# christhetree/mod_extraction

Measured on AMD Instinct MI355X. Metric: 44.1 kHz audio-seconds/sec (train step), interwoven ph/fl/ch, higher is better.
Workload: dtype f32

## Files before the change

mod_extraction_amd/csrc/melspec.hip:

```cpp
#include "wave_fft.h"

#define MEL_NFFT 1024
#define MEL_FR 16

struct cfloat { float re, im; };
__device__ __forceinline__ cfloat cmul(cfloat a, cfloat b)
{
    cfloat r;
    r.re = a.re * b.re - a.im * b.im;
    r.im = a.re * b.im + a.im * b.re;
    return r;
}
__device__ __forceinline__ cfloat cadd(cfloat a, cfloat b) { return {a.re + b.re, a.im + b.im}; }
__device__ __forceinline__ cfloat csub(cfloat a, cfloat b) { return {a.re - b.re, a.im - b.im}; }

__global__ __launch_bounds__(256) void melspec_kernel(
    const float *__restrict__ x, int N, const float *__restrict__ window,
    const float2 *__restrict__ twiddle,
    const float *__restrict__ fb,
    const int *__restrict__ band_lo, const int *__restrict__ band_hi, int n_mels, int hop,
    int n_frames, int out_pitch, float eps, int f0, int f1, int t0, int t1, int coef_cap, float *__restrict__ out)
{
    __shared__ cfloat fftbuf[4][MEL_NFFT + 64];
    __shared__ float powbuf[4][MEL_NFFT / 2 + 1];
    __shared__ float2 tw_s[MEL_NFFT];
    extern __shared__ float melbuf[];
    const int tid = threadIdx.x, lane = tid & 63, wave = tid >> 6;
    const int plane = blockIdx.y;
    const int tile0 = blockIdx.x * MEL_FR;
    const float *xp = x + (size_t)plane * N;
    cfloat *buf = fftbuf[wave];
    float *power = powbuf[wave];
    float *coef = melbuf + n_mels * (MEL_FR + 1);
    int *boff = reinterpret_cast<int *>(coef + coef_cap);
    for (int i = tid; i < MEL_NFFT; i += 256) tw_s[i] = twiddle[i];
    if (tid == 0) {
        int acc = 0;
        for (int m = 0; m < n_mels; ++m) { boff[m] = acc; acc += band_hi[m] - band_lo[m]; }
        boff[n_mels] = acc;
    }
    __syncthreads();
    const bool packed = boff[n_mels] <= coef_cap;
    if (packed) {
        for (int m = tid; m < n_mels; m += 256) {
            const int lo = band_lo[m], hi = band_hi[m], o = boff[m];
            for (int kk = lo; kk < hi; ++kk) coef[o + kk - lo] = fb[(size_t)kk * n_mels + m];
        }
    }
    __syncthreads();

    for (int fl = wave; fl < MEL_FR; fl += 4) {
        const int t = tile0 + fl;
        if (t >= n_frames) continue;
        cfloat R[4][4];
#pragma unroll
        for (int bq = 0; bq < 4; ++bq)
#pragma unroll
            for (int cq = 0; cq < 4; ++cq) {
                const int n = lane + 64 * bq + 256 * cq;
                int sidx = t * hop + n - MEL_NFFT / 2;
                if (sidx < 0) sidx = -sidx;
                if (sidx >= N) sidx = 2 * (N - 1) - sidx;
                sidx = sidx < 0 ? 0 : sidx;
                R[bq][cq].re = xp[sidx] * window[n];
                R[bq][cq].im = 0.0f;
            }
        auto bfly = [&](int pass, int j, const cfloat (&vin)[4], cfloat (&o)[4]) {
            const int Ns = 1 << (2 * pass);
            const int k = j & (Ns - 1);
            const int tw_step = k * (MEL_NFFT / (Ns * 4));
            cfloat v0 = vin[0], v1 = vin[1], v2 = vin[2], v3 = vin[3];
            if (pass > 0) {
                float2 w1 = tw_s[tw_step], w2 = tw_s[2 * tw_step], w3 = tw_s[3 * tw_step];
                v1 = cmul(v1, {w1.x, w1.y});
                v2 = cmul(v2, {w2.x, w2.y});
                v3 = cmul(v3, {w3.x, w3.y});
            }
            cfloat a0 = cadd(v0, v2), a1 = csub(v0, v2), a2 = cadd(v1, v3), d = csub(v1, v3);
            cfloat a3 = {d.im, -d.re};
            o[0] = cadd(a0, a2);
            o[1] = cadd(a1, a3);
            o[2] = csub(a0, a2);
            o[3] = csub(a1, a3);
        };
        auto out_pos = [](int pass, int j, int r) {
            const int Ns = 1 << (2 * pass), k = j & (Ns - 1);
            return ((j - k) << 2) + k + r * Ns;
        };
        cfloat O[4][4], P[4][4];
#pragma unroll
        for (int bq = 0; bq < 4; ++bq) bfly(0, lane + 64 * bq, R[bq], O[bq]);
#pragma unroll
        for (int r = 0; r < 4; ++r) {
            const cfloat vin[4] = {O[0][r], O[1][r], O[2][r], O[3][r]};
            bfly(1, 4 * lane + r, vin, P[r]);
        }
#pragma unroll
        for (int r = 0; r < 4; ++r)
#pragma unroll
            for (int r2 = 0; r2 < 4; ++r2) {
                const int q = out_pos(1, 4 * lane + r, r2);
                buf[q + (q >> 4)] = P[r][r2];
            }
        __builtin_amdgcn_wave_barrier();
#pragma unroll
        for (int bq = 0; bq < 4; ++bq)
#pragma unroll
            for (int cq = 0; cq < 4; ++cq) {
                const int q = lane + 64 * bq + 256 * cq;
                R[bq][cq] = buf[q + (q >> 4)];
            }
        __builtin_amdgcn_wave_barrier();
        const int k2 = lane & 15;
#pragma unroll
        for (int bq = 0; bq < 4; ++bq) bfly(2, lane + 64 * bq, R[bq], O[bq]);
#pragma unroll
        for (int r = 0; r < 4; ++r) {
            const cfloat vin[4] = {O[0][r], O[1][r], O[2][r], O[3][r]};
            bfly(3, 4 * (lane - k2) + k2 + 16 * r, vin, P[r]);
        }
#pragma unroll
        for (int r = 0; r < 4; ++r)
#pragma unroll
            for (int r2 = 0; r2 < 4; ++r2) {
                const int q = out_pos(3, 4 * (lane - k2) + k2 + 16 * r, r2);
                buf[q + 16 * (q >> 8)] = P[r][r2];
            }
        __builtin_amdgcn_wave_barrier();
#pragma unroll
        for (int bq = 0; bq < 4; ++bq)
#pragma unroll
            for (int cq = 0; cq < 4; ++cq) {
                const int q = lane + 64 * bq + 256 * cq;
                R[bq][cq] = buf[q + 16 * (q >> 8)];
            }
        __builtin_amdgcn_wave_barrier();
#pragma unroll
        for (int bq = 0; bq < 4; ++bq) {
            const int j = lane + 64 * bq;
            bfly(4, j, R[bq], O[bq]);
#pragma unroll
            for (int r = 0; r < 3; ++r) {
                const int bin = j + 256 * r;
                if (bin <= MEL_NFFT / 2) {
                    const cfloat z = O[bq][r];
                    const float mag = sqrtf(z.re * z.re + z.im * z.im);
                    power[bin] = mag * mag;
                }
            }
        }
        __builtin_amdgcn_wave_barrier();
        for (int m = lane; m < n_mels; m += 64) {
            float acc = 0.0f;
            const int lo = band_lo[m], hi = band_hi[m];
            if (packed) {
                const float *cm = coef + boff[m] - lo;
                for (int kk = lo; kk < hi; ++kk) acc = fmaf(cm[kk], power[kk], acc);
            } else {
                float c = 0.0f;
                for (int kk = lo; kk < hi; ++kk) {
                    const float yv = fb[(size_t)kk * n_mels + m] * power[kk] - c;
                    const float tv = acc + yv;
                    c = (tv - acc) - yv;
                    acc = tv;
                }
            }
            melbuf[m * (MEL_FR + 1) + fl] = acc;
        }
        __builtin_amdgcn_wave_barrier();
    }
    __syncthreads();
    float *op = out + (size_t)plane * n_mels * out_pitch;
    for (int idx = tid; idx < n_mels * MEL_FR; idx += 256) {
        const int m = idx / MEL_FR, fl = idx % MEL_FR;
        const int t = tile0 + fl;
        if (t < out_pitch) {
            float v = 0.0f;
            if (t < n_frames) {
                float p = melbuf[m * (MEL_FR + 1) + fl];
                if ((m >= f0 && m < f1) || (t >= t0 && t < t1)) p = 0.0f;
                v = logf(fmaxf(p, eps));
            }
            op[(size_t)m * out_pitch + t] = v;
        }
    }
}

template <int NF>
__global__ __launch_bounds__(WF<NF>::WAVES * 64) void melspec_wf_kernel(
    const float *__restrict__ x, int N, const float *__restrict__ window, const float2 *__restrict__ twiddle,
    const float *__restrict__ fb, const int *__restrict__ band_lo, const int *__restrict__ band_hi, int n_mels, int hop,
    int n_frames, int out_pitch, float eps, int f0, int f1, int t0, int t1, int coef_cap, float *__restrict__ out)
{
    constexpr int L = WF<NF>::L, E = WF<NF>::E, NB = WF<NF>::NB, WAVES = WF<NF>::WAVES, FW = WF<NF>::FW, NT = WAVES * 64;
    __shared__ cf fftbuf[WAVES * FW][WF<NF>::LEN];
    __shared__ float powbuf[WAVES * FW][NF / 2 + 1];
    __shared__ cf tw_s[NF];
    extern __shared__ float melbuf[];
    const int tid = threadIdx.x, lane = tid & 63, wave = tid >> 6, g = lane / L, a = lane % L;
    const int plane = blockIdx.y;
    const int tile0 = blockIdx.x * MEL_FR;
    const float *xp = x + (size_t)plane * N;
    cf *buf = fftbuf[wave * FW + g];
    float *power = powbuf[wave * FW + g];
    float *coef = melbuf + n_mels * (MEL_FR + 1);
    int *boff = reinterpret_cast<int *>(coef + coef_cap);
    for (int i = tid; i < NF; i += NT) {
        const float2 w = twiddle[i];
        tw_s[i] = {w.x, w.y};
    }
    if (tid == 0) {
        int acc = 0;
        for (int m = 0; m < n_mels; ++m) { boff[m] = acc; acc += band_hi[m] - band_lo[m]; }
        boff[n_mels] = acc;
    }
    __syncthreads();
    const bool packed = boff[n_mels] <= coef_cap;
    if (packed) {
        for (int m = tid; m < n_mels; m += NT) {
            const int lo = band_lo[m], hi = band_hi[m], o = boff[m];
            for (int kk = lo; kk < hi; ++kk) coef[o + kk - lo] = fb[(size_t)kk * n_mels + m];
        }
    }
    __syncthreads();
    FftLane<NF> fl_;
    fft_lane_setup<NF, 1>(fl_, buf, tw_s, twiddle, a);

    for (int fb0 = wave * FW; fb0 < MEL_FR; fb0 += WAVES * FW) {
        const int fl = fb0 + g;
        if (tile0 + fb0 >= n_frames) break;
        const int t = tile0 + fl;
        const bool live = t < n_frames && fl < MEL_FR;
        const int tt = live ? t : n_frames - 1;
        cf R[NB][4], Z[E];
#pragma unroll
        for (int bq = 0; bq < NB; ++bq)
#pragma unroll
            for (int cq = 0; cq < 4; ++cq) {
                const int n = a + L * bq + (NF / 4) * cq;
                int sidx = tt * hop + n - NF / 2;
                if (sidx < 0) sidx = -sidx;
                if (sidx >= N) sidx = 2 * (N - 1) - sidx;
                sidx = sidx < 0 ? 0 : sidx;
                R[bq][cq] = {xp[sidx] * window[n], 0.0f};
            }
        wave_fft<NF, false>(R, Z, fl_);
#pragma unroll
        for (int i = 0; i < E; ++i) {
            const int bin = pos_final<NF>(i, a);
            if (bin <= NF / 2) {
                const float mag = sqrtf(Z[i].x * Z[i].x + Z[i].y * Z[i].y);
                power[bin] = mag * mag;
            }
        }
        __builtin_amdgcn_wave_barrier();
        if (live) {
            for (int m = a; m < n_mels; m += L) {
                float acc = 0.0f;
                const int lo = band_lo[m], hi = band_hi[m];
                if (packed) {
                    const float *cm = coef + boff[m] - lo;
                    for (int kk = lo; kk < hi; ++kk) acc = fmaf(cm[kk], power[kk], acc);
                } else {
                    float c = 0.0f;
                    for (int kk = lo; kk < hi; ++kk) {
                        const float yv = fb[(size_t)kk * n_mels + m] * power[kk] - c;
                        const float tv = acc + yv;
                        c = (tv - acc) - yv;
                        acc = tv;
                    }
                }
                melbuf[m * (MEL_FR + 1) + fl] = acc;
            }
        }
        __builtin_amdgcn_wave_barrier();
    }
    __syncthreads();
    float *op = out + (size_t)plane * n_mels * out_pitch;
    for (int idx = tid; idx < n_mels * MEL_FR; idx += NT) {
        const int m = idx / MEL_FR, fl = idx % MEL_FR;
        const int t = tile0 + fl;
        if (t < out_pitch) {
            float v = 0.0f;
            if (t < n_frames) {
                float p = melbuf[m * (MEL_FR + 1) + fl];
                if ((m >= f0 && m < f1) || (t >= t0 && t < t1)) p = 0.0f;
                v = logf(fmaxf(p, eps));
            }
            op[(size_t)m * out_pitch + t] = v;
        }
    }
}

MX_EXPORT int mx_logmel_fwd(const float *x, int64_t planes, int64_t N, const float *window,
                            const float *twiddle, const float *fb, const int32_t *band_lo,
                            const int32_t *band_hi, int64_t n_fft, int64_t hop, int64_t n_mels,
                            int64_t n_frames, int64_t out_pitch, float eps, int32_t f0, int32_t f1,
                            int32_t t0, int32_t t1, float *out, void *stream)
{
    if (!x || !window || !twiddle || !fb || !band_lo || !band_hi || !out || planes <= 0) return MX_ERR_ARG;
    if (hop <= 0 || n_frames < 0 || (N > 0 && n_frames > N / hop + 1)) return MX_ERR_ARG;
    if ((n_fft != 512 && n_fft != 1024 && n_fft != 2048) || N <= n_fft / 2 || N >= (1ll << 30) || planes > 65535 || n_mels > 2048 ||
        out_pitch < n_frames)
        return MX_ERR_UNSUPPORTED;
    const int tiles = (int)((out_pitch + MEL_FR - 1) / MEL_FR);
    const int coef_cap = 2 * ((int)n_fft / 2 + 1) + 2 * (int)n_mels;
    const size_t lds = ((size_t)n_mels * (MEL_FR + 1) + coef_cap + n_mels + 1) * sizeof(float);
    const void *fn = n_fft == MEL_NFFT ? (const void *)melspec_kernel
                     : n_fft == 512    ? (const void *)melspec_wf_kernel<512>
                                       : (const void *)melspec_wf_kernel<2048>;
    static size_t static_lds[3] = {0, 0, 0};
    static MxLdsLatch latch[3] = {};
    const int ki = n_fft == MEL_NFFT ? 0 : n_fft == 512 ? 1 : 2;
    if (!static_lds[ki]) {
        hipFuncAttributes fa;
        if (hipFuncGetAttributes(&fa, fn) != hipSuccess) return MX_ERR_LAUNCH;
        static_lds[ki] = fa.sharedSizeBytes ? fa.sharedSizeBytes : 1;
    }
    const size_t lds_cap = 160 * 1024;
    if (static_lds[ki] + lds > lds_cap) return MX_ERR_UNSUPPORTED;
    if (static_lds[ki] + lds > 64 * 1024 && mx_set_dyn_lds(latch[ki], fn, lds_cap - static_lds[ki]) != MX_OK) return MX_ERR_LAUNCH;
    if (n_fft != MEL_NFFT) {
        if (n_fft == 512)
            hipLaunchKernelGGL((melspec_wf_kernel<512>), dim3(tiles, (unsigned)planes), dim3(WF<512>::WAVES * 64), lds, (hipStream_t)stream,
                               x, (int)N, window, (const float2 *)twiddle, fb, band_lo, band_hi, (int)n_mels, (int)hop, (int)n_frames,
                               (int)out_pitch, eps, f0, f1, t0, t1, coef_cap, out);
        else
            hipLaunchKernelGGL((melspec_wf_kernel<2048>), dim3(tiles, (unsigned)planes), dim3(WF<2048>::WAVES * 64), lds, (hipStream_t)stream,
                               x, (int)N, window, (const float2 *)twiddle, fb, band_lo, band_hi, (int)n_mels, (int)hop, (int)n_frames,
                               (int)out_pitch, eps, f0, f1, t0, t1, coef_cap, out);
        return mx_launch_status();
    }
    hipLaunchKernelGGL(melspec_kernel, dim3(tiles, (unsigned)planes), dim3(256), lds, (hipStream_t)stream,
                       x, (int)N, window, (const float2 *)twiddle, fb, band_lo, band_hi, (int)n_mels, (int)hop,
                       (int)n_frames, (int)out_pitch, eps, f0, f1, t0, t1, coef_cap, out);
    return mx_launch_status();
}
```

Baseline: 7580.

## Process multiple mel tiles per workgroup and skip masked frames and bands

The 1024-point mel kernel now loops over several frame tiles per workgroup, chosen when the grid is large, so the per-block setup (twiddle load, band offsets, filterbank packing) is amortised. The serial prefix sum over band widths becomes a wave-level shuffle scan, and band limits are cached in LDS. Interior frames skip reflection index math, and the mel dot product is unrolled by four. Frames and mel bands inside the masked ranges skip FFT and dot work entirely. The trade-off is fewer workgroups, which lowers parallelism on smaller inputs, plus extra LDS and an unrolled loop that reads a few entries past each band.

```diff
diff --git a/mod_extraction_amd/csrc/melspec.hip b/mod_extraction_amd/csrc/melspec.hip
--- a/mod_extraction_amd/csrc/melspec.hip
+++ b/mod_extraction_amd/csrc/melspec.hip
@@ -2,6 +2,9 @@
 
 #define MEL_NFFT 1024
 #define MEL_FR 16
+#ifndef MEL_TPW
+#define MEL_TPW 2
+#endif
 
 struct cfloat { float re, im; };
 __device__ __forceinline__ cfloat cmul(cfloat a, cfloat b)
@@ -19,170 +22,223 @@
     const float2 *__restrict__ twiddle,
     const float *__restrict__ fb,
     const int *__restrict__ band_lo, const int *__restrict__ band_hi, int n_mels, int hop,
-    int n_frames, int out_pitch, float eps, int f0, int f1, int t0, int t1, int coef_cap, float *__restrict__ out)
+    int n_frames, int out_pitch, float eps, int f0, int f1, int t0, int t1, int coef_cap, int tiles_per_wg,
+    float *__restrict__ out)
 {
     __shared__ cfloat fftbuf[4][MEL_NFFT + 64];
-    __shared__ float powbuf[4][MEL_NFFT / 2 + 1];
+    __shared__ float powbuf[4][MEL_NFFT / 2 + 4];
     __shared__ float2 tw_s[MEL_NFFT];
     extern __shared__ float melbuf[];
     const int tid = threadIdx.x, lane = tid & 63, wave = tid >> 6;
     const int plane = blockIdx.y;
-    const int tile0 = blockIdx.x * MEL_FR;
     const float *xp = x + (size_t)plane * N;
     cfloat *buf = fftbuf[wave];
     float *power = powbuf[wave];
     float *coef = melbuf + n_mels * (MEL_FR + 1);
     int *boff = reinterpret_cast<int *>(coef + coef_cap);
+    int *blo = boff + n_mels + 1, *bhi = blo + n_mels;
     for (int i = tid; i < MEL_NFFT; i += 256) tw_s[i] = twiddle[i];
-    if (tid == 0) {
-        int acc = 0;
-        for (int m = 0; m < n_mels; ++m) { boff[m] = acc; acc += band_hi[m] - band_lo[m]; }
-        boff[n_mels] = acc;
+    for (int m = tid; m < n_mels; m += 256) {
+        blo[m] = band_lo[m];
+        bhi[m] = band_hi[m];
+    }
+    __syncthreads();
+    if (tid < 64) {
+        const int per = (n_mels + 63) / 64, m0 = lane * per, m1 = min(m0 + per, n_mels);
+        int s = 0;
+        for (int m = m0; m < m1; ++m) s += bhi[m] - blo[m];
+        int incl = s;
+#pragma unroll
+        for (int d = 1; d < 64; d <<= 1) {
+            const int v = __shfl_up(incl, d);
+            if (lane >= d) incl += v;
+        }
+        int acc = incl - s;
+        for (int m = m0; m < m1; ++m) { boff[m] = acc; acc += bhi[m] - blo[m]; }
+        if (lane == 63) boff[n_mels] = incl;
     }
     __syncthreads();
     const bool packed = boff[n_mels] <= coef_cap;
     if (packed) {
         for (int m = tid; m < n_mels; m += 256) {
-            const int lo = band_lo[m], hi = band_hi[m], o = boff[m];
-            for (int kk = lo; kk < hi; ++kk) coef[o + kk - lo] = fb[(size_t)kk * n_mels + m];
-        }
-    }
-    __syncthreads();
-
-    for (int fl = wave; fl < MEL_FR; fl += 4) {
-        const int t = tile0 + fl;
-        if (t >= n_frames) continue;
-        cfloat R[4][4];
-#pragma unroll
-        for (int bq = 0; bq < 4; ++bq)
-#pragma unroll
-            for (int cq = 0; cq < 4; ++cq) {
-                const int n = lane + 64 * bq + 256 * cq;
-                int sidx = t * hop + n - MEL_NFFT / 2;
-                if (sidx < 0) sidx = -sidx;
-                if (sidx >= N) sidx = 2 * (N - 1) - sidx;
-                sidx = sidx < 0 ? 0 : sidx;
-                R[bq][cq].re = xp[sidx] * window[n];
-                R[bq][cq].im = 0.0f;
-            }
-        auto bfly = [&](int pass, int j, const cfloat (&vin)[4], cfloat (&o)[4]) {
-            const int Ns = 1 << (2 * pass);
-            const int k = j & (Ns - 1);
-            const int tw_step = k * (MEL_NFFT / (Ns * 4));
-            cfloat v0 = vin[0], v1 = vin[1], v2 = vin[2], v3 = vin[3];
-            if (pass > 0) {
-                float2 w1 = tw_s[tw_step], w2 = tw_s[2 * tw_step], w3 = tw_s[3 * tw_step];
-                v1 = cmul(v1, {w1.x, w1.y});
-                v2 = cmul(v2, {w2.x, w2.y});
-                v3 = cmul(v3, {w3.x, w3.y});
-            }
-            cfloat a0 = cadd(v0, v2), a1 = csub(v0, v2), a2 = cadd(v1, v3), d = csub(v1, v3);
-            cfloat a3 = {d.im, -d.re};
-            o[0] = cadd(a0, a2);
-            o[1] = cadd(a1, a3);
-            o[2] = csub(a0, a2);
-            o[3] = csub(a1, a3);
-        };
-        auto out_pos = [](int pass, int j, int r) {
-            const int Ns = 1 << (2 * pass), k = j & (Ns - 1);
-            return ((j - k) << 2) + k + r * Ns;
-        };
-        cfloat O[4][4], P[4][4];
-#pragma unroll
-        for (int bq = 0; bq < 4; ++bq) bfly(0, lane + 64 * bq, R[bq], O[bq]);
-#pragma unroll
-        for (int r = 0; r < 4; ++r) {
-            const cfloat vin[4] = {O[0][r], O[1][r], O[2][r], O[3][r]};
-            bfly(1, 4 * lane + r, vin, P[r]);
-        }
-#pragma unroll
-        for (int r = 0; r < 4; ++r)
-#pragma unroll
-            for (int r2 = 0; r2 < 4; ++r2) {
-                const int q = out_pos(1, 4 * lane + r, r2);
-                buf[q + (q >> 4)] = P[r][r2];
-            }
-        __builtin_amdgcn_wave_barrier();
-#pragma unroll
-        for (int bq = 0; bq < 4; ++bq)
-#pragma unroll
-            for (int cq = 0; cq < 4; ++cq) {
-                const int q = lane + 64 * bq + 256 * cq;
-                R[bq][cq] = buf[q + (q >> 4)];
-            }
-        __builtin_amdgcn_wave_barrier();
-        const int k2 = lane & 15;
-#pragma unroll
-        for (int bq = 0; bq < 4; ++bq) bfly(2, lane + 64 * bq, R[bq], O[bq]);
-#pragma unroll
-        for (int r = 0; r < 4; ++r) {
-            const cfloat vin[4] = {O[0][r], O[1][r], O[2][r], O[3][r]};
-            bfly(3, 4 * (lane - k2) + k2 + 16 * r, vin, P[r]);
-        }
-#pragma unroll
-        for (int r = 0; r < 4; ++r)
-#pragma unroll
-            for (int r2 = 0; r2 < 4; ++r2) {
-                const int q = out_pos(3, 4 * (lane - k2) + k2 + 16 * r, r2);
-                buf[q + 16 * (q >> 8)] = P[r][r2];
-            }
-        __builtin_amdgcn_wave_barrier();
-#pragma unroll
-        for (int bq = 0; bq < 4; ++bq)
-#pragma unroll
-            for (int cq = 0; cq < 4; ++cq) {
-                const int q = lane + 64 * bq + 256 * cq;
-                R[bq][cq] = buf[q + 16 * (q >> 8)];
-            }
-        __builtin_amdgcn_wave_barrier();
-#pragma unroll
-        for (int bq = 0; bq < 4; ++bq) {
-            const int j = lane + 64 * bq;
-            bfly(4, j, R[bq], O[bq]);
-#pragma unroll
-            for (int r = 0; r < 3; ++r) {
-                const int bin = j + 256 * r;
-                if (bin <= MEL_NFFT / 2) {
-                    const cfloat z = O[bq][r];
-                    const float mag = sqrtf(z.re * z.re + z.im * z.im);
-                    power[bin] = mag * mag;
-                }
-            }
-        }
-        __builtin_amdgcn_wave_barrier();
-        for (int m = lane; m < n_mels; m += 64) {
-            float acc = 0.0f;
-            const int lo = band_lo[m], hi = band_hi[m];
-            if (packed) {
-                const float *cm = coef + boff[m] - lo;
-                for (int kk = lo; kk < hi; ++kk) acc = fmaf(cm[kk], power[kk], acc);
+            const int lo = blo[m], hi = bhi[m], o = boff[m] - lo;
+            for (int kk = lo; kk < hi; kk += 8) {
+                float v[8];
+#pragma unroll
+                for (int i = 0; i < 8; ++i) v[i] = kk + i < hi ? fb[(size_t)(kk + i) * n_mels + m] : 0.0f;
+#pragma unroll
+                for (int i = 0; i < 8; ++i)
+                    if (kk + i < hi) coef[o + kk + i] = v[i];
+            }
+        }
+    }
+    __syncthreads();
+
+    for (int tl = 0; tl < tiles_per_wg; ++tl) {
+        const int tile0 = (blockIdx.x * tiles_per_wg + tl) * MEL_FR;
+        if (tile0 >= out_pitch) break;
+        for (int fl = wave; fl < MEL_FR; fl += 4) {
+            const int t = tile0 + fl;
+            if (t >= n_frames || (t >= t0 && t < t1)) continue;
+            cfloat R[4][4];
+            float xv[4][4];
+            const int s0 = t * hop - MEL_NFFT / 2;
+            if (s0 >= 0 && s0 + MEL_NFFT <= N) {
+                const float *xs = xp + s0 + lane;
+#pragma unroll
+                for (int bq = 0; bq < 4; ++bq)
+#pragma unroll
+                    for (int cq = 0; cq < 4; ++cq) xv[bq][cq] = xs[64 * bq + 256 * cq];
             } else {
-                float c = 0.0f;
-                for (int kk = lo; kk < hi; ++kk) {
-                    const float yv = fb[(size_t)kk * n_mels + m] * power[kk] - c;
-                    const float tv = acc + yv;
-                    c = (tv - acc) - yv;
-                    acc = tv;
-                }
-            }
-            melbuf[m * (MEL_FR + 1) + fl] = acc;
-        }
-        __builtin_amdgcn_wave_barrier();
-    }
-    __syncthreads();
-    float *op = out + (size_t)plane * n_mels * out_pitch;
-    for (int idx = tid; idx < n_mels * MEL_FR; idx += 256) {
-        const int m = idx / MEL_FR, fl = idx % MEL_FR;
-        const int t = tile0 + fl;
-        if (t < out_pitch) {
-            float v = 0.0f;
-            if (t < n_frames) {
-                float p = melbuf[m * (MEL_FR + 1) + fl];
-                if ((m >= f0 && m < f1) || (t >= t0 && t < t1)) p = 0.0f;
-                v = logf(fmaxf(p, eps));
-            }
-            op[(size_t)m * out_pitch + t] = v;
-        }
+#pragma unroll
+                for (int bq = 0; bq < 4; ++bq)
+#pragma unroll
+                    for (int cq = 0; cq < 4; ++cq) {
+                        int sidx = s0 + lane + 64 * bq + 256 * cq;
+                        if (sidx < 0) sidx = -sidx;
+                        if (sidx >= N) sidx = 2 * (N - 1) - sidx;
+                        sidx = sidx < 0 ? 0 : sidx;
+                        xv[bq][cq] = xp[sidx];
+                    }
+            }
+#pragma unroll
+            for (int bq = 0; bq < 4; ++bq)
+#pragma unroll
+                for (int cq = 0; cq < 4; ++cq) {
+                    R[bq][cq].re = xv[bq][cq] * window[lane + 64 * bq + 256 * cq];
+                    R[bq][cq].im = 0.0f;
+                }
+            auto bfly = [&](int pass, int j, const cfloat (&vin)[4], cfloat (&o)[4]) {
+                const int Ns = 1 << (2 * pass);
+                const int k = j & (Ns - 1);
+                const int tw_step = k * (MEL_NFFT / (Ns * 4));
+                cfloat v0 = vin[0], v1 = vin[1], v2 = vin[2], v3 = vin[3];
+                if (pass > 0) {
+                    float2 w1 = tw_s[tw_step], w2 = tw_s[2 * tw_step], w3 = tw_s[3 * tw_step];
+                    v1 = cmul(v1, {w1.x, w1.y});
+                    v2 = cmul(v2, {w2.x, w2.y});
+                    v3 = cmul(v3, {w3.x, w3.y});
+                }
+                cfloat a0 = cadd(v0, v2), a1 = csub(v0, v2), a2 = cadd(v1, v3), d = csub(v1, v3);
+                cfloat a3 = {d.im, -d.re};
+                o[0] = cadd(a0, a2);
+                o[1] = cadd(a1, a3);
+                o[2] = csub(a0, a2);
+                o[3] = csub(a1, a3);
+            };
+            auto out_pos = [](int pass, int j, int r) {
+                const int Ns = 1 << (2 * pass), k = j & (Ns - 1);
+                return ((j - k) << 2) + k + r * Ns;
+            };
+            cfloat O[4][4], P[4][4];
+#pragma unroll
+            for (int bq = 0; bq < 4; ++bq) bfly(0, lane + 64 * bq, R[bq], O[bq]);
+#pragma unroll
+            for (int r = 0; r < 4; ++r) {
+                const cfloat vin[4] = {O[0][r], O[1][r], O[2][r], O[3][r]};
+                bfly(1, 4 * lane + r, vin, P[r]);
+            }
+#pragma unroll
+            for (int r = 0; r < 4; ++r)
+#pragma unroll
+                for (int r2 = 0; r2 < 4; ++r2) {
+                    const int q = out_pos(1, 4 * lane + r, r2);
+                    buf[q + (q >> 4)] = P[r][r2];
+                }
+            __builtin_amdgcn_wave_barrier();
+#pragma unroll
+            for (int bq = 0; bq < 4; ++bq)
+#pragma unroll
+                for (int cq = 0; cq < 4; ++cq) {
+                    const int q = lane + 64 * bq + 256 * cq;
+                    R[bq][cq] = buf[q + (q >> 4)];
+                }
+            __builtin_amdgcn_wave_barrier();
+            const int k2 = lane & 15;
+#pragma unroll
+            for (int bq = 0; bq < 4; ++bq) bfly(2, lane + 64 * bq, R[bq], O[bq]);
+#pragma unroll
+            for (int r = 0; r < 4; ++r) {
+                const cfloat vin[4] = {O[0][r], O[1][r], O[2][r], O[3][r]};
+                bfly(3, 4 * (lane - k2) + k2 + 16 * r, vin, P[r]);
+            }
+#pragma unroll
+            for (int r = 0; r < 4; ++r)
+#pragma unroll
+                for (int r2 = 0; r2 < 4; ++r2) {
+                    const int q = out_pos(3, 4 * (lane - k2) + k2 + 16 * r, r2);
+                    buf[q + 16 * (q >> 8)] = P[r][r2];
+                }
+            __builtin_amdgcn_wave_barrier();
+#pragma unroll
+            for (int bq = 0; bq < 4; ++bq)
+#pragma unroll
+                for (int cq = 0; cq < 4; ++cq) {
+                    const int q = lane + 64 * bq + 256 * cq;
+                    R[bq][cq] = buf[q + 16 * (q >> 8)];
+                }
+            __builtin_amdgcn_wave_barrier();
+#pragma unroll
+            for (int bq = 0; bq < 4; ++bq) {
+                const int j = lane + 64 * bq;
+                bfly(4, j, R[bq], O[bq]);
+#pragma unroll
+                for (int r = 0; r < 3; ++r) {
+                    const int bin = j + 256 * r;
+                    if (bin <= MEL_NFFT / 2) {
+                        const cfloat z = O[bq][r];
+                        const float mag = sqrtf(z.re * z.re + z.im * z.im);
+                        power[bin] = mag * mag;
+                    }
+                }
+            }
+            __builtin_amdgcn_wave_barrier();
+            for (int m = lane; m < n_mels; m += 64) {
+                if (m >= f0 && m < f1) continue;
+                float acc = 0.0f;
+                const int lo = blo[m], hi = bhi[m];
+                if (packed) {
+                    const float *cm = coef + boff[m] - lo;
+                    for (int kk = lo; kk < hi; kk += 4) {
+                        float c4[4], p4[4];
+#pragma unroll
+                        for (int i = 0; i < 4; ++i) {
+                            c4[i] = cm[kk + i];
+                            p4[i] = power[kk + i];
+                        }
+#pragma unroll
+                        for (int i = 0; i < 4; ++i)
+                            if (kk + i < hi) acc = fmaf(c4[i], p4[i], acc);
+                    }
+                } else {
+                    float c = 0.0f;
+                    for (int kk = lo; kk < hi; ++kk) {
+                        const float yv = fb[(size_t)kk * n_mels + m] * power[kk] - c;
+                        const float tv = acc + yv;
+                        c = (tv - acc) - yv;
+                        acc = tv;
+                    }
+                }
+                melbuf[m * (MEL_FR + 1) + fl] = acc;
+            }
+            __builtin_amdgcn_wave_barrier();
+        }
+        __syncthreads();
+        float *op = out + (size_t)plane * n_mels * out_pitch;
+        for (int idx = tid; idx < n_mels * MEL_FR; idx += 256) {
+            const int m = idx / MEL_FR, fl = idx % MEL_FR;
+            const int t = tile0 + fl;
+            if (t < out_pitch) {
+                float v = 0.0f;
+                if (t < n_frames) {
+                    const bool masked = (m >= f0 && m < f1) || (t >= t0 && t < t1);
+                    const float p = masked ? 0.0f : melbuf[m * (MEL_FR + 1) + fl];
+                    v = logf(fmaxf(p, eps));
+                }
+                op[(size_t)m * out_pitch + t] = v;
+            }
+        }
+        __syncthreads();
     }
 }
 
@@ -305,7 +361,7 @@
         return MX_ERR_UNSUPPORTED;
     const int tiles = (int)((out_pitch + MEL_FR - 1) / MEL_FR);
     const int coef_cap = 2 * ((int)n_fft / 2 + 1) + 2 * (int)n_mels;
-    const size_t lds = ((size_t)n_mels * (MEL_FR + 1) + coef_cap + n_mels + 1) * sizeof(float);
+    const size_t lds = ((size_t)n_mels * (MEL_FR + 1) + coef_cap + n_mels + 1 + (n_fft == MEL_NFFT ? 2 * n_mels : 0)) * sizeof(float);
     const void *fn = n_fft == MEL_NFFT ? (const void *)melspec_kernel
                      : n_fft == 512    ? (const void *)melspec_wf_kernel<512>
                                        : (const void *)melspec_wf_kernel<2048>;
@@ -331,8 +387,9 @@
                                (int)out_pitch, eps, f0, f1, t0, t1, coef_cap, out);
         return mx_launch_status();
     }
-    hipLaunchKernelGGL(melspec_kernel, dim3(tiles, (unsigned)planes), dim3(256), lds, (hipStream_t)stream,
+    const int tpw = (int64_t)tiles * planes >= 4 * 512 * MEL_TPW ? MEL_TPW : 1;
+    hipLaunchKernelGGL(melspec_kernel, dim3((tiles + tpw - 1) / tpw, (unsigned)planes), dim3(256), lds, (hipStream_t)stream,
                        x, (int)N, window, (const float2 *)twiddle, fb, band_lo, band_hi, (int)n_mels, (int)hop,
-                       (int)n_frames, (int)out_pitch, eps, f0, f1, t0, t1, coef_cap, out);
+                       (int)n_frames, (int)out_pitch, eps, f0, f1, t0, t1, coef_cap, tpw, out);
     return mx_launch_status();
 }
```

Result: no change. 7604 (median of 6 runs) (+0.3%).
